# yewzijian/RegTR

Measured on NVIDIA H100. Metric: pairs/sec on 3DMatch-size clouds (~20k pts); pose err vs ref, higher is better.
Workload: dtype f32

## Files before the change

include/regtr_b200.h:

```cpp
#ifndef REGTR_B200_H_
#define REGTR_B200_H_

#include <stddef.h>
#include <stdint.h>

#ifdef __cplusplus
extern "C" {
#endif

#define REGTR_OK 0
#define REGTR_ERR_ARG (-1)
#define REGTR_ERR_WORKSPACE (-2)
#define REGTR_ERR_UNSUPPORTED (-3)

#define REGTR_STATUS_KEY_RANGE 1u
#define REGTR_STATUS_CAPACITY 2u
#define REGTR_STATUS_GRID 4u
#define REGTR_STATUS_RANGE 8u

int regtr_version(void);
const char* regtr_build_info(void);


size_t regtr_grid_subsample_ws_bytes(int n_cap, int n_clouds);
size_t regtr_grid_subsample_state_bytes(int n_cap);
int regtr_grid_subsample(const float* xyz, const int32_t* offs, int n_clouds, int n_cap, float dl,
                         float* out_xyz, int out_cap, int32_t* out_offs, uint32_t* status,
                         void* ws, size_t ws_bytes, void* state, size_t state_bytes, void* stream);
size_t regtr_grid_subsample_sorted_ws_bytes(int n_cap);
int regtr_grid_subsample_sorted(const float* xyz, const int32_t* offs, int n_clouds, int n_cap, float dl,
                                float* out_xyz, int out_cap, int32_t* out_offs, uint32_t* status,
                                void* ws, size_t ws_bytes, void* stream);

size_t regtr_cellgrid_bytes(int n_cap);
size_t regtr_cellgrid_ws_bytes(int n_cap);
size_t regtr_cellgrid_state_bytes(int n_cap);
int regtr_cellgrid_build(const float* xyz, const int32_t* offs, int n_clouds, int n_cap, float cell,
                         void* grid, int32_t* order, uint32_t* status,
                         void* ws, size_t ws_bytes, void* state, size_t state_bytes, void* stream);

int regtr_ball_query(const float* q, const int32_t* q_offs, const int32_t* q_order,
                     const float* s, const int32_t* s_offs, const void* s_grid,
                     int n_clouds, int nq_cap, int s_cap, int K, float radius,
                     int32_t* out_idx32, int64_t* out_idx64, void* stream);


size_t regtr_kpconv_ws_bytes(int Nq, int Ns, int Cin);
size_t regtr_kpconv_fwd_ws_bytes(int Nq, int Ns, int Cin, int Cout);
int regtr_kpconv_fwd(const float* q, const float* s, const int32_t* idx, const float* x,
                     const float* W, const float* kp, int Nq, int Ns, const int32_t* nq_dev,
                     const int32_t* ns_dev, int K, int Cin, int Cout,
                     float extent, float* out, void* ws, size_t ws_bytes, void* stream);

int regtr_kpconv_aggregate(const float* q, const float* s, const int32_t* idx, const float* x,
                           const float* kp, int Nq, int Ns, const int32_t* nq_dev, const int32_t* ns_dev,
                           int K, int Cin, float extent,
                           float* wf, uint8_t* rowflag_ws, int flags_ready, void* stream);

int regtr_max_pool(const float* x, const int32_t* idx, int Nq, int Ns, const int32_t* ns_dev, int K, int C,
                   float* out, void* stream);

size_t regtr_instnorm_ws_bytes(int n_cap, int n_clouds, int C);
size_t regtr_instnorm_counter_bytes(int n_clouds, int C);
int regtr_instnorm_act(const float* x, const int32_t* offs, int n_clouds, int n_cap, int C, float eps,
                       const float* res, float slope, float* out, uint8_t* rowflag_out,
                       void* ws, size_t ws_bytes, int32_t* counters, void* stream);

int regtr_instnorm_apply(const float* x, const int32_t* offs, int n_clouds, int n_cap, int C, const float* stats,
                         const float* res, float slope, float* out, uint8_t* rowflag_out, void* stream);


int regtr_split_tf32(const float* x, long long n, float* hi, float* lo, void* stream);

size_t regtr_gemm_ws_bytes(int M, int N, int K);
int regtr_gemm_tf32x3(const float* A, int lda, const float* B_hi, const float* B_lo, int ldb,
                      float* C, int ldc, const float* bias, const float* R, int ldr,
                      int M, int N, int K, const int32_t* m_dev, int relu,
                      void* ws, size_t ws_bytes, void* stream);

size_t regtr_instnorm_part_bytes(int M, int N);
int regtr_gemm_tf32x3_instats(const float* A, int lda, const float* B_hi, const float* B_lo, int ldb,
                              float* C, int ldc, int M, int N, int K, const int32_t* m_dev,
                              const int32_t* offs, int n_clouds, float eps, void* part, float* stats,
                              void* ws, size_t ws_bytes, void* stream);


int regtr_pos_embed_sine(const float* xyz, int n, const float* dim_t, int n_freq, int d_model,
                         float scale, float* out, void* stream);

int regtr_layernorm_pos(const float* x, const float* gamma, const float* beta, const float* pos,
                        int n, const int32_t* n_dev, int E, float eps, float* y, float* y_pos, void* stream);

int regtr_attention_plan(const int32_t* offs, int B, int32_t* plan, void* stream);

int regtr_mha_varlen_fwd(const float* Q, int ldq, const float* K, int ldk, const float* V, int ldv,
                         float* O, int ldo, const int32_t* q_start, const int32_t* q_len,
                         const int32_t* k_start, const int32_t* k_len, int n_problems,
                         int max_q_len, const int32_t* tile_base, int max_tiles,
                         int n_heads, int head_dim, float scale, void* stream);

int regtr_corr_decode_fwd(const float* Qp, const float* Kp, int ld, const float* xyz, float* out,
                          const int32_t* q_start, const int32_t* q_len, const int32_t* k_start,
                          const int32_t* k_len, int n_problems, int max_q_len, int n_layers, int n_rows,
                          int D, float scale, void* stream);

int regtr_gemm_tf32x3_qkv_bf16(const float* A, int lda, const float* B_hi, const float* B_lo, int ldb,
                               const float* bias, int M, int N, int K, int split, void* qk_out, int ld_qk,
                               void* vt_out, int ld_vt, const int32_t* m_dev, void* stream);
int regtr_mha_bf16_tc_fwd(const void* QK, int ld_qk, const void* Vt, int ld_vt, int n_tokens, float* O,
                          int ldo, const int32_t* q_start, const int32_t* q_len, const int32_t* k_start,
                          const int32_t* k_len, int n_problems, int max_q_len, int n_heads, int head_dim,
                          float scale, void* stream);

int regtr_gemm_tf32x3_qkv_split(const float* A, int lda, const float* B_hi, const float* B_lo, int ldb,
                                const float* bias, int M, int N, int K, int E, float qscale, float* qk4, int ld4,
                                float* vt2, int ld_vt, const int32_t* m_dev, void* stream);
int regtr_mha_tf32_tc_fwd(const float* qk4, int ld4, const float* vt2, int ld_vt, int n_tokens, float* O, int ldo,
                          const int32_t* q_start, const int32_t* q_len, const int32_t* k_start,
                          const int32_t* k_len, int n_problems, int max_q_len, const int32_t* tile_base,
                          int max_tiles, int n_heads, int head_dim, void* stream);

int regtr_mha_varlen_fwd_lse(const float* Q, int ldq, const float* K, int ldk, const float* V, int ldv,
// ... 175 lines not shown
```

regtr_b200/csrc/gemm_tc.cu:

```cuda
#include <cuda_bf16.h>


#include "common.cuh"
#include <stdlib.h>

#include "tc.cuh"

namespace {

struct QkvOut {
    __nv_bfloat16* qk;
    int ld_qk;
    __nv_bfloat16* vt;
    int ld_vt;
    int split;
    float* qk4;
    int ld4;
    float* vt2;
    int ld_vtf;
    int E;
    float qscale;
};
constexpr QkvOut NO_QKV = {nullptr, 0, nullptr, 0, 0, nullptr, 0, nullptr, 0, 0, 0.f};


template <int OFF>
__device__ __forceinline__ void transpose_sum_step(float (&v)[32], int lane) {
    const bool up = (lane & OFF) != 0;
#pragma unroll
    for (int i = 0; i < OFF; ++i) {
        const float mine = up ? v[i + OFF] : v[i];
        const float give = up ? v[i] : v[i + OFF];
        v[i] = mine + __shfl_xor_sync(0xffffffffu, give, OFF);
    }
    if constexpr (OFF > 1) transpose_sum_step<OFF / 2>(v, lane);
}
__device__ __forceinline__ float warp_transpose_sum(float (&v)[32], int lane) {
    transpose_sum_step<16>(v, lane);
    return v[0];
}

__global__ void __launch_bounds__(256)
k_in_finalize_part(const float2* __restrict__ part, const float* __restrict__ C, int ldc, const int32_t* __restrict__ offs,
                   int N, float eps, int direct_all, float2* __restrict__ stats) {
    __shared__ double red[8][32][2];
    const int c = blockIdx.x, col = blockIdx.y * 32 + threadIdx.x, w = threadIdx.y;
    const int a = offs[c], b = offs[c + 1];
    int g_lo = (a + 31) >> 5, g_hi = b >> 5;
    const bool full = !direct_all && g_lo < g_hi;
    const int head_end = full ? 32 * g_lo : b, tail_start = full ? 32 * g_hi : b;
    double s = 0.0, q = 0.0, k0 = 0.0;
    if (col < N && b > a) {
        k0 = (double)C[(size_t)a * ldc + col];
        if (full)
            for (int g = g_lo + w; g < g_hi; g += 8) {
                const float2 p = part[(size_t)g * N + col];
                const double d = (double)C[(size_t)g * 32 * ldc + col] - k0;
                s += (double)p.x + 32.0 * d;
                q += (double)p.y + d * (2.0 * (double)p.x + 32.0 * d);
            }
        for (int r = a + w; r < head_end; r += 8) { const double v = (double)C[(size_t)r * ldc + col] - k0; s += v; q += v * v; }
        for (int r = tail_start + w; r < b; r += 8) { const double v = (double)C[(size_t)r * ldc + col] - k0; s += v; q += v * v; }
    }
    red[w][threadIdx.x][0] = s; red[w][threadIdx.x][1] = q;
    __syncthreads();
    if (w == 0 && col < N) {
        for (int t = 1; t < 8; ++t) { s += red[t][threadIdx.x][0]; q += red[t][threadIdx.x][1]; }
        const int n = b - a;
        const double dn = n > 0 ? (double)n : 1.0;
        const double shift = s / dn;
        double var = q / dn - shift * shift;
        var = var > 0.0 ? var : 0.0;
        stats[(size_t)c * N + col] = make_float2((float)(k0 + shift), (float)(1.0 / sqrt(var + (double)eps)));
    }
}

constexpr int BM = 128;
constexpr int BK = 32;
constexpr uint32_t HI_MASK = 0xFFFFE000u;

__device__ __forceinline__ float tf32_hi(float x) { return regtr_tf32_rne(x); }

__global__ void k_split_tf32(const float* __restrict__ x, long long n, float* __restrict__ hi, float* __restrict__ lo) {
    const long long i = (long long)blockIdx.x * blockDim.x + threadIdx.x;
    if (i >= n) return;
    const float v = x[i], h = tf32_hi(v);
    hi[i] = h;
    lo[i] = tf32_hi(v - h);
}

constexpr int CONSUMER_THREADS = 256;
constexpr int GEMM_THREADS = CONSUMER_THREADS + 32;

template <int BN, int ST> struct CfgT {
    static constexpr int STAGES = ST;
    static constexpr int A_BYTES = BM * BK * 4;
    static constexpr int B_BYTES = BN * BK * 4;
    static constexpr int STAGE_BYTES = A_BYTES + 2 * B_BYTES;
    static constexpr int LDT = BN + 4;
    static constexpr int TILE_BYTES = BM * LDT * 4;
    static constexpr int SMEM = STAGES * STAGE_BYTES + TILE_BYTES + 1024  + 256 ;
    static constexpr int MIN_CTAS = SMEM <= 113 * 1024 ? 2 : 1;
};

__device__ __forceinline__ void consumer_sync() { asm volatile("bar.sync 1, %0;" ::"n"(CONSUMER_THREADS) : "memory"); }

template <int BN>
__device__ __forceinline__ void wgmma_tf32(float* d, const uint32_t* a, uint64_t bdesc, uint32_t accumulate) {
    if constexpr (BN == 128) tc::wgmma_tf32_n128(d, a, bdesc, accumulate);
    else if constexpr (BN == 64) tc::wgmma_tf32_n64(d, a, bdesc, accumulate);
    else tc::wgmma_tf32_n32(d, a, bdesc, accumulate);
}

template <int BN, int ST>
__global__ void __launch_bounds__(GEMM_THREADS, CfgT<BN, ST>::MIN_CTAS)
// ... 481 lines not shown
```

regtr_b200/csrc/norm.cu:

```cuda
#include "common.cuh"

namespace {

constexpr int IN_CH = 128;
constexpr int IN_TY = 8;
constexpr int IN_CT = 128;

__device__ __forceinline__ bool chunk_of(const int32_t* __restrict__ offs, int n_clouds, int chunk, int& cloud,
                                         int& r0, int& r1, int& first, int& count) {
    int acc = 0;
    for (int c = 0; c < n_clouds; ++c) {
        const int a = offs[c], b = offs[c + 1];
        const int nc = (b - a + IN_CH - 1) / IN_CH;
        if (chunk < acc + nc) {
            cloud = c;
            r0 = a + (chunk - acc) * IN_CH;
            r1 = min(r0 + IN_CH, b);
            first = acc;
            count = nc;
            return true;
        }
        acc += nc;
    }
    return false;
// ... 55 lines not shown
                fs[j] += p.x; fss[j] += p.y;
            }
    }
#pragma unroll
    for (int j = 0; j < 4; ++j) { red[threadIdx.y][threadIdx.x][j] = fs[j]; red[threadIdx.y][threadIdx.x][4 + j] = fss[j]; }
    __syncthreads();
    if (threadIdx.y == 0 && c < C) {
        for (int t = 1; t < IN_TY; ++t)
#pragma unroll
            for (int j = 0; j < 4; ++j) { fs[j] += red[t][threadIdx.x][j]; fss[j] += red[t][threadIdx.x][4 + j]; }
        const int n = offs[cloud + 1] - offs[cloud];
        const double dn = n > 0 ? (double)n : 1.0;
#pragma unroll
        for (int j = 0; j < 4; ++j) {
            const double mean = fs[j] / dn;
            double var = fss[j] / dn - mean * mean;
            var = var > 0.0 ? var : 0.0;
            stats[(size_t)cloud * C + c + j] = make_float2((float)mean, (float)(1.0 / sqrt(var + (double)eps)));
        }
    }
}

__global__ void __launch_bounds__(32 * IN_TY)
k_in_finalize(const int32_t* __restrict__ offs, int n_clouds, int C, float eps, const double2* __restrict__ partial,
              float2* __restrict__ stats) {
    __shared__ double2 red[IN_TY][32];
    const int cloud = blockIdx.x;
    const int c = blockIdx.y * 32 + threadIdx.x;
    int first = 0;
    for (int k = 0; k < cloud; ++k) first += (offs[k + 1] - offs[k] + IN_CH - 1) / IN_CH;
    const int n = offs[cloud + 1] - offs[cloud];
    const int nc = (n + IN_CH - 1) / IN_CH;
    double s = 0.0, ss = 0.0;
    if (c < C) {
        for (int t = threadIdx.y; t < nc; t += IN_TY) {
            const double2 p = partial[(size_t)(first + t) * C + c];
            s += p.x; ss += p.y;
        }
    }
    red[threadIdx.y][threadIdx.x] = make_double2(s, ss);
    __syncthreads();
    if (threadIdx.y == 0 && c < C) {
        for (int t = 1; t < IN_TY; ++t) { s += red[t][threadIdx.x].x; ss += red[t][threadIdx.x].y; }
        const double dn = n > 0 ? (double)n : 1.0;
        const double mean = s / dn;
        double var = ss / dn - mean * mean;
        var = var > 0.0 ? var : 0.0;
        stats[(size_t)cloud * C + c] = make_float2((float)mean, (float)(1.0 / sqrt(var + (double)eps)));
    }
}

template <bool FLAGS>
__global__ void k_in_apply(const float* x, const int32_t* __restrict__ offs, int n_clouds, int n_cap, int C,
                           const float2* __restrict__ stats, const float* res, float slope, float* out,
                           uint8_t* __restrict__ flags) {
    const int c4n = C >> 2;
    const int n_real = offs[n_clouds];
    const unsigned total = (unsigned)min(n_cap, (n_real + 127) & ~127) * (unsigned)c4n;
    const unsigned stride = gridDim.x * blockDim.x;
    for (unsigned t0 = blockIdx.x * blockDim.x; t0 < total; t0 += stride) {
        const unsigned t = t0 + threadIdx.x;
        const bool in_range = t < total;
        int r = 0, c = 0;
        if (in_range) { regtr_row_col(t, (unsigned)c4n, r, c); c *= 4; }
        const size_t o = (size_t)r * C + c;
        const bool live = in_range && r < n_real;
        float y[4] = {0.f, 0.f, 0.f, 0.f};
        if (live) {
            const float4 v = *reinterpret_cast<const float4*>(x + o);
            float4 rv = make_float4(0.f, 0.f, 0.f, 0.f);
            if (res) rv = *reinterpret_cast<const float4*>(res + o);
            const int cloud = regtr_cloud_of(offs, n_clouds, r);
            const float4 st01 = *reinterpret_cast<const float4*>(stats + (size_t)cloud * C + c);
            const float4 st23 = *reinterpret_cast<const float4*>(stats + (size_t)cloud * C + c + 2);
            y[0] = (v.x - st01.x) * st01.y + rv.x; y[1] = (v.y - st01.z) * st01.w + rv.y;
            y[2] = (v.z - st23.x) * st23.y + rv.z; y[3] = (v.w - st23.z) * st23.w + rv.w;
            if (slope >= 0.f) {
#pragma unroll
                for (int j = 0; j < 4; ++j) y[j] = y[j] > 0.f ? y[j] : y[j] * slope;
            }
        }
        if (in_range) *reinterpret_cast<float4*>(out + o) = make_float4(y[0], y[1], y[2], y[3]);
        if (FLAGS) {
            double acc = ((double)y[0] + (double)y[1]) + ((double)y[2] + (double)y[3]);
            for (int d = 1; d < c4n; d <<= 1) acc += __shfl_xor_sync(0xffffffffu, acc, d);
            if (in_range && (threadIdx.x & (c4n - 1)) == 0) flags[r] = live && acc > 0.0;
        }
    }
}

template <int PER>
__global__ void k_layernorm_pos(const float* __restrict__ x, const float* __restrict__ gamma,
                                const float* __restrict__ beta, const float* __restrict__ pos, int n,
                                const int32_t* __restrict__ n_dev, int E, float eps, float* __restrict__ y,
                                float* __restrict__ y_pos) {
    const int row = (blockIdx.x * blockDim.x + threadIdx.x) >> 5, lane = threadIdx.x & 31;
    if (n_dev) n = min(n, *n_dev);
    if (row >= n) return;
    const float* xr = x + (size_t)row * E;
    const int per = E / 32;
    float v[PER], gm[PER], bt[PER], ps[PER];
#pragma unroll
    for (int j = 0; j < PER; ++j)
        if (j < per) {
            const int c = j * 32 + lane;
            v[j] = xr[c]; gm[j] = __ldg(gamma + c); bt[j] = __ldg(beta + c);
            ps[j] = (y_pos && pos) ? pos[(size_t)row * E + c] : 0.f;
        }
    float s = 0.f;
#pragma unroll
    for (int j = 0; j < PER; ++j) if (j < per) s += v[j];
    const float mean = warp_sum(s) / (float)E;
    float ss = 0.f;
#pragma unroll
    for (int j = 0; j < PER; ++j) if (j < per) { const float d = v[j] - mean; ss += d * d; }
    const float rstd = 1.f / sqrtf(warp_sum(ss) / (float)E + eps);
#pragma unroll
    for (int j = 0; j < PER; ++j) {
        if (j >= per) break;
        const int c = j * 32 + lane;
        const float o = (v[j] - mean) * rstd * gm[j] + bt[j];
        if (y) y[(size_t)row * E + c] = o;
        if (y_pos) y_pos[(size_t)row * E + c] = o + ps[j];
    }
}
// ... 6 lines not shown
    regtr_row_col((unsigned)t, (unsigned)d_model, i, c);
    float o = 0.f;
    if (c < 3 * n_freq) {
        const int a = c / n_freq, f = c % n_freq;
        const float v = __fdiv_rn(__fmul_rn(xyz[3 * i + a], scale), dim_t[f]);
        o = (f & 1) ? cosf(v) : sinf(v);
    }
    out[t] = o;
}

static inline int in_apply_grid(long long items) {
    const long long b = (items + 255) / 256;
    return (int)(b < 8 * REGTR_NUM_SMS ? (b > 0 ? b : 1) : 8 * REGTR_NUM_SMS);
}

}

extern "C" {

static inline int in_chunks(int n_cap, int n_clouds) { return regtr_cdiv(n_cap > 0 ? n_cap : 1, IN_CH) + n_clouds; }

size_t regtr_instnorm_ws_bytes(int n_cap, int n_clouds, int C) {
    const size_t c = (size_t)(C > 0 ? C : 1), nc = (size_t)(n_clouds > 0 ? n_clouds : 1);
    return regtr_align((size_t)in_chunks(n_cap, (int)nc) * c * sizeof(double2)) + regtr_align(nc * c * sizeof(float2));
}

size_t regtr_instnorm_counter_bytes(int n_clouds, int C) {
    return sizeof(int32_t) * (size_t)(n_clouds > 0 ? n_clouds : 1) * (size_t)regtr_cdiv(C > 0 ? C : 1, IN_CT);
}

int regtr_instnorm_act(const float* x, const int32_t* offs, int n_clouds, int n_cap, int C, float eps,
                       const float* res, float slope, float* out, uint8_t* rowflag_out, void* ws, size_t ws_bytes,
                       int32_t* counters, void* stream_) {
    cudaStream_t st = (cudaStream_t)stream_;
    if (!offs || n_clouds <= 0 || n_cap < 0 || C <= 0) return REGTR_ERR_ARG;
    if (C % 4 != 0 || (long long)n_cap * (C / 4) >= (1ll << 31)) return REGTR_ERR_UNSUPPORTED;
    if (n_cap == 0) return REGTR_OK;
    if (!x || !out || !ws) return REGTR_ERR_ARG;
    if (ws_bytes < regtr_instnorm_ws_bytes(n_cap, n_clouds, C)) return REGTR_ERR_WORKSPACE;
    const int chunks = in_chunks(n_cap, n_clouds);
    double2* partial = (double2*)ws;
    float2* stats = (float2*)((char*)ws + regtr_align((size_t)chunks * C * sizeof(double2)));
    dim3 block(32, IN_TY);
    k_in_stats<<<dim3(chunks, regtr_cdiv(C, IN_CT)), block, 0, st>>>(x, offs, n_clouds, C, partial, counters, eps, stats);
    REGTR_CHECK_LAUNCH();
    if (!counters) {
        k_in_finalize<<<dim3(n_clouds, regtr_cdiv(C, 32)), block, 0, st>>>(offs, n_clouds, C, eps, partial, stats);
        REGTR_CHECK_LAUNCH();
    }
    if (rowflag_out) {
        const int c4n = C / 4;
        if (c4n > 32 || (c4n & (c4n - 1))) return REGTR_ERR_UNSUPPORTED;
        k_in_apply<true><<<in_apply_grid((long long)n_cap * c4n), 256, 0, st>>>(x, offs, n_clouds, n_cap, C, stats,
                                                                                  res, slope, out, rowflag_out);
    } else {
        k_in_apply<false><<<in_apply_grid((long long)n_cap * (C / 4)), 256, 0, st>>>(x, offs, n_clouds, n_cap, C,
                                                                                      stats, res, slope, out, nullptr);
    }
    REGTR_CHECK_LAUNCH();
    return REGTR_OK;
}

int regtr_instnorm_apply(const float* x, const int32_t* offs, int n_clouds, int n_cap, int C, const float* stats,
                         const float* res, float slope, float* out, uint8_t* rowflag_out, void* stream_) {
    cudaStream_t st = (cudaStream_t)stream_;
    if (!offs || n_clouds <= 0 || n_cap < 0 || C <= 0) return REGTR_ERR_ARG;
    if (C % 4 != 0 || (long long)n_cap * (C / 4) >= (1ll << 31)) return REGTR_ERR_UNSUPPORTED;
    if (n_cap == 0) return REGTR_OK;
    if (!x || !out || !stats) return REGTR_ERR_ARG;
    const float2* stp = reinterpret_cast<const float2*>(stats);
    if (rowflag_out) {
        const int c4n = C / 4;
        if (c4n > 32 || (c4n & (c4n - 1))) return REGTR_ERR_UNSUPPORTED;
        k_in_apply<true><<<in_apply_grid((long long)n_cap * c4n), 256, 0, st>>>(x, offs, n_clouds, n_cap, C, stp, res, slope,
                                                                                  out, rowflag_out);
    } else {
        k_in_apply<false><<<in_apply_grid((long long)n_cap * (C / 4)), 256, 0, st>>>(x, offs, n_clouds, n_cap, C, stp, res,
                                                                                      slope, out, nullptr);
    }
    REGTR_CHECK_LAUNCH();
    return REGTR_OK;
}

int regtr_layernorm_pos(const float* x, const float* gamma, const float* beta, const float* pos, int n,
                        const int32_t* n_dev, int E, float eps, float* y, float* y_pos, void* stream_) {
    cudaStream_t st = (cudaStream_t)stream_;
    if (n < 0 || E <= 0 || E % 32 != 0 || E > 1024) return REGTR_ERR_ARG;
    if (n == 0) return REGTR_OK;
    if (!x || !gamma || !beta || (!y && !y_pos)) return REGTR_ERR_ARG;
    if (E <= 256)
        k_layernorm_pos<8><<<regtr_cdiv((long long)n * 32, 256), 256, 0, st>>>(x, gamma, beta, pos, n, n_dev, E, eps, y, y_pos);
    else
        k_layernorm_pos<32><<<regtr_cdiv((long long)n * 32, 256), 256, 0, st>>>(x, gamma, beta, pos, n, n_dev, E, eps, y, y_pos);
    REGTR_CHECK_LAUNCH();
    return REGTR_OK;
}

int regtr_pos_embed_sine(const float* xyz, int n, const float* dim_t, int n_freq, int d_model, float scale,
                         float* out, void* stream_) {
    cudaStream_t st = (cudaStream_t)stream_;
    if (n < 0 || n_freq <= 0 || d_model < 3 * n_freq) return REGTR_ERR_ARG;
    if ((long long)n * d_model >= (1ll << 31)) return REGTR_ERR_UNSUPPORTED;
    if (n == 0) return REGTR_OK;
    if (!xyz || !dim_t || !out) return REGTR_ERR_ARG;
    k_pos_embed_sine<<<regtr_cdiv((long long)n * d_model, 256), 256, 0, st>>>(xyz, n, dim_t, n_freq, d_model, scale, out);
    REGTR_CHECK_LAUNCH();
    return REGTR_OK;
}

}
```

regtr_b200/kpconv.py:

```python
from __future__ import annotations

import logging
from typing import List

import torch
import torch.nn as nn
import torch.nn.functional as F

from . import ops
from .config import pyramid_plan
from .lazy import LazyDict
from .weights import kernel_disposition

_CELL_SLACK = 1.0001



def level_capacities(cfg, cap0: int, ratio: float = 0.40, quantum: int = 256):
    levels, _, _ = pyramid_plan(cfg)
    caps = [int(cap0)]
    for _ in levels[1:]:
        c = int(caps[-1] * ratio) + 1
        caps.append(min(caps[-1], (c + quantum - 1) // quantum * quantum))
    return caps
# ... 167 lines not shown
    return ops.max_pool(x.contiguous(), inds if inds.dtype == torch.int32 else inds.to(torch.int32))


class KPConv(nn.Module):

    def __init__(self, kernel_size, p_dim, in_channels, out_channels, KP_extent, radius,
                 fixed_kernel_points='center', KP_influence='linear', aggregation_mode='sum',
                 deformable=False, modulated=False):
        super().__init__()
        if deformable or modulated:
            raise NotImplementedError('deformable / modulated KPConv is outside the hot path')
        if KP_influence != 'linear' or aggregation_mode != 'sum':
            raise NotImplementedError("only KP_influence='linear', aggregation_mode='sum' are on the hot path")
        if kernel_size != 15 or p_dim != 3:
            raise NotImplementedError('the fused kernel is specialised for 15 kernel points in 3-D')
        self.K, self.p_dim = kernel_size, p_dim
        self.in_channels, self.out_channels = in_channels, out_channels
        self.radius, self.KP_extent = radius, KP_extent
        self.weights = nn.Parameter(torch.empty((kernel_size, in_channels, out_channels), dtype=torch.float32))
        bound = 1.0 / (in_channels * out_channels) ** 0.5
        nn.init.uniform_(self.weights, -bound, bound)
        self.kernel_points = nn.Parameter(torch.from_numpy(kernel_disposition(radius, kernel_size)),
                                          requires_grad=False)

    def forward(self, q_pts, s_pts, neighb_inds, x, nq_dev=None, ns_dev=None, row_flags=None, instats=None):
        idx = neighb_inds if neighb_inds.dtype == torch.int32 else neighb_inds.to(torch.int32)
        return ops.kpconv(q_pts.contiguous(), s_pts.contiguous(), idx.contiguous(), x.contiguous(),
                          self.weights, self.kernel_points, self.KP_extent, nq_dev=nq_dev, ns_dev=ns_dev,
                          row_flags=row_flags, instats=instats)

    def __repr__(self):
        return 'KPConv(radius: {:.2f}, extent: {:.2f}, in_feat: {:d}, out_feat: {:d})'.format(
            self.radius, self.KP_extent, self.in_channels, self.out_channels)


class BatchNormBlock(nn.Module):

    def __init__(self, in_dim, use_bn, bn_momentum):
        super().__init__()
        self.in_dim, self.use_bn, self.bn_momentum = in_dim, use_bn, bn_momentum
        if not use_bn:
            self.bias = nn.Parameter(torch.zeros(in_dim, dtype=torch.float32))

    def fuse(self, x, offs, n_clouds, res=None, slope=-1.0, want_flags=False):
        if self.use_bn:
            return ops.instnorm_act(x, offs, n_clouds, res=res, slope=slope, want_flags=want_flags)
        if want_flags:
            raise NotImplementedError('row flags are only fused into the InstanceNorm pass')
        y = x + self.bias
        if res is not None:
            y = y + res
        return F.leaky_relu(y, slope) if slope >= 0 else y

    def apply(self, x, stats, offs, n_clouds, res=None, slope=-1.0, want_flags=False):
        return ops.instnorm_apply(x, offs, n_clouds, stats, res=res, slope=slope, want_flags=want_flags)

    def forward(self, x, stack_lengths):
        offs = ops.make_offsets(stack_lengths, x.device)
        return self.fuse(x.contiguous(), offs, offs.numel() - 1)


class UnaryBlock(nn.Module):

    def __init__(self, in_dim, out_dim, use_bn, bn_momentum, no_relu=False):
        super().__init__()
        self.in_dim, self.out_dim, self.use_bn, self.no_relu = in_dim, out_dim, use_bn, no_relu
        self.mlp = nn.Linear(in_dim, out_dim, bias=False)
        self.batch_norm = BatchNormBlock(out_dim, use_bn, bn_momentum)

    def fuse(self, x, offs, n_clouds, res=None, final_slope=None, m_dev=None, want_flags=False, skip=False):
        slope = final_slope if final_slope is not None else (-1.0 if self.no_relu else 0.1)
        if self.use_bn and self.out_dim % 32 == 0 and EPILOGUE_STATS:
            y, stats, *xs = ops.linear_instats(x, self.mlp.weight, offs, n_clouds, m_dev=m_dev, skip=skip)
            out = self.batch_norm.apply(y, stats, offs, n_clouds, res=res, slope=slope, want_flags=want_flags)
        else:
            xs = [x]
            out = self.batch_norm.fuse(ops.linear(x, self.mlp.weight, m_dev=m_dev), offs, n_clouds, res=res,
                                       slope=slope, want_flags=want_flags)
        if not skip:
            return out
        return (*out, xs[0]) if want_flags else (out, xs[0])

    def forward(self, x, stack_lengths=None):
        offs = ops.make_offsets(stack_lengths, x.device)
        return self.fuse(x, offs, offs.numel() - 1)


def _block_io(block, batch):
    m = _meta_private(batch, batch['points'][0].device if 'points' in batch else batch['_points'][0].device)
    li = block.layer_ind
    pts, offs, nd = m['_points'], m['_offs'], m['_ndev']
    if 'strided' in block.block_name:
        return (pts[li + 1], pts[li], m['_pools32'][li], offs[li], offs[li + 1],
                nd[li + 1] if nd else None, nd[li] if nd else None, m['_n_clouds'])
    return (pts[li], pts[li], m['_neighbors32'][li], offs[li], offs[li],
            nd[li] if nd else None, nd[li] if nd else None, m['_n_clouds'])


class SimpleBlock(nn.Module):

    def __init__(self, block_name, in_dim, out_dim, radius, layer_ind, config):
        super().__init__()
        self.block_name, self.layer_ind = block_name, layer_ind
        self.in_dim, self.out_dim = in_dim, out_dim
        extent = radius * config.KP_extent / config.conv_radius
        self.KPConv = KPConv(config.num_kernel_points, config.in_points_dim, in_dim, out_dim // 2, extent, radius,
                             fixed_kernel_points=config.fixed_kernel_points, KP_influence=config.KP_influence,
                             aggregation_mode=config.aggregation_mode, deformable='deform' in block_name,
                             modulated=config.modulated)
        self.batch_norm = BatchNormBlock(out_dim // 2, config.use_batch_norm, config.batch_norm_momentum)

    def forward(self, x, batch):
        q, s, idx, _, offs_post, nq_dev, ns_dev, nc = _block_io(self, batch)
        y = self.KPConv(q, s, idx, x, nq_dev, ns_dev)
        return self.batch_norm.fuse(y, offs_post, nc, slope=0.1)


class ResnetBottleneckBlock(nn.Module):

    def __init__(self, block_name, in_dim, out_dim, radius, layer_ind, config):
        super().__init__()
        self.block_name, self.layer_ind = block_name, layer_ind
        self.in_dim, self.out_dim = in_dim, out_dim
        bn, mom = config.use_batch_norm, config.batch_norm_momentum
        self.use_bn = bn
        extent = radius * config.KP_extent / config.conv_radius
        mid = out_dim // 4
        self.unary1 = UnaryBlock(in_dim, mid, bn, mom) if in_dim != mid else nn.Identity()
        self.KPConv = KPConv(config.num_kernel_points, config.in_points_dim, mid, mid, extent, radius,
                             fixed_kernel_points=config.fixed_kernel_points, KP_influence=config.KP_influence,
                             aggregation_mode=config.aggregation_mode, deformable='deform' in block_name,
                             modulated=config.modulated)
        self.batch_norm_conv = BatchNormBlock(mid, bn, mom)
        self.unary2 = UnaryBlock(mid, out_dim, bn, mom, no_relu=True)
        self.unary_shortcut = UnaryBlock(in_dim, out_dim, bn, mom, no_relu=True) if in_dim != out_dim \
            else nn.Identity()

    def forward(self, features, batch):
        q, s, idx, offs_pre, offs_post, nq_dev, ns_dev, nc = _block_io(self, batch)
        flags = None
        if isinstance(self.unary1, UnaryBlock) and self.use_bn:
            x, flags, features = self.unary1.fuse(features, offs_pre, nc, m_dev=ns_dev, want_flags=True, skip=True)
        else:
            x = self.unary1.fuse(features, offs_pre, nc, m_dev=ns_dev) if isinstance(self.unary1, UnaryBlock) \
                else features
        if self.use_bn and self.KPConv.out_channels % 32 == 0 and EPILOGUE_STATS:
            x, stats = self.KPConv(q, s, idx, x, nq_dev, ns_dev, row_flags=flags, instats=(offs_post, nc))
            x = self.batch_norm_conv.apply(x, stats, offs_post, nc, slope=0.1)
        else:
            x = self.KPConv(q, s, idx, x, nq_dev, ns_dev, row_flags=flags)
            x = self.batch_norm_conv.fuse(x, offs_post, nc, slope=0.1)
        shortcut = ops.max_pool(features, idx, ns_dev) if 'strided' in self.block_name else features
        if isinstance(self.unary_shortcut, UnaryBlock):
            shortcut = self.unary_shortcut.fuse(shortcut, offs_post, nc, m_dev=nq_dev)
        return self.unary2.fuse(x, offs_post, nc, res=shortcut, final_slope=0.1, m_dev=nq_dev)


def block_decider(block_name, radius, in_dim, out_dim, layer_ind, config):
    if block_name in ('simple', 'simple_strided'):
        return SimpleBlock(block_name, in_dim, out_dim, radius, layer_ind, config)
    if block_name in ('resnetb', 'resnetb_strided'):
        return ResnetBottleneckBlock(block_name, in_dim, out_dim, radius, layer_ind, config)
    raise NotImplementedError(f'block {block_name!r} is outside the RegTR hot path (SURVEY.md 2 row 3)')


class KPFEncoder(nn.Module):

    def __init__(self, config, d_bottle, increase_channel_when_downsample=True):
        super().__init__()
        self.logger = logging.getLogger(__name__)
        octave = 0
        r = config.first_subsampling_dl * config.conv_radius
        in_dim, out_dim = config.in_feats_dim, config.first_feats_dim
        self.encoder_blocks = nn.ModuleList()
        self.encoder_skip_dims, self.encoder_skips = [], []
        block = None
        for block_i, block in enumerate(config.architecture):
            if any(t in block for t in ('pool', 'strided', 'upsample', 'global')):
                self.encoder_skips.append(block_i)
                self.encoder_skip_dims.append(in_dim)
            if 'upsample' in block:
                break
            self.encoder_blocks.append(block_decider(block, r, in_dim, out_dim, octave, config))
            in_dim = out_dim // 2 if 'simple' in block else out_dim
            if 'pool' in block or 'strided' in block:
                octave += 1
                r *= 2
                if increase_channel_when_downsample:
                    out_dim *= 2
        if 'upsample' not in block:
            self.encoder_skips.append(block_i)
            self.encoder_skip_dims.append(in_dim)

    def forward(self, x, batch):
        skip_x = []
        for block_i, block_op in enumerate(self.encoder_blocks):
            if block_i in self.encoder_skips:
                skip_x.append(x)
            x = block_op(x, batch)
        return x, skip_x
```

regtr_b200/lib.py:

```python
from __future__ import annotations

import ctypes
import os
import re

import torch

HERE = os.path.dirname(os.path.abspath(__file__))
LIB_PATH = os.path.join(HERE, 'libregtr_b200.so')
HEADER = os.path.join(os.path.dirname(HERE), 'include', 'regtr_b200.h')


class RegtrLibError(RuntimeError):
    pass


_c = ctypes
_P = _c.c_void_p
_I = _c.c_int
_F = _c.c_float
_Z = _c.c_size_t

SIGNATURES = {
    'regtr_version': (_I, []),
    'regtr_build_info': (_c.c_char_p, []),
    'regtr_grid_subsample_ws_bytes': (_Z, [_I, _I]),
    'regtr_grid_subsample_state_bytes': (_Z, [_I]),
    'regtr_grid_subsample': (_I, [_P, _P, _I, _I, _F, _P, _I, _P, _P, _P, _Z, _P, _Z, _P]),
    'regtr_grid_subsample_sorted_ws_bytes': (_Z, [_I]),
    'regtr_grid_subsample_sorted': (_I, [_P, _P, _I, _I, _F, _P, _I, _P, _P, _P, _Z, _P]),
    'regtr_cellgrid_bytes': (_Z, [_I]),
    'regtr_cellgrid_ws_bytes': (_Z, [_I]),
    'regtr_cellgrid_state_bytes': (_Z, [_I]),
    'regtr_cellgrid_build': (_I, [_P, _P, _I, _I, _F, _P, _P, _P, _P, _Z, _P, _Z, _P]),
    'regtr_ball_query': (_I, [_P, _P, _P, _P, _P, _P, _I, _I, _I, _I, _F, _P, _P, _P]),
    'regtr_kpconv_ws_bytes': (_Z, [_I, _I, _I]),
    'regtr_kpconv_fwd_ws_bytes': (_Z, [_I, _I, _I, _I]),
    'regtr_kpconv_fwd': (_I, [_P, _P, _P, _P, _P, _P, _I, _I, _P, _P, _I, _I, _I, _F, _P, _P, _Z, _P]),
    'regtr_kpconv_aggregate': (_I, [_P, _P, _P, _P, _P, _I, _I, _P, _P, _I, _I, _F, _P, _P, _I, _P]),
    'regtr_max_pool': (_I, [_P, _P, _I, _I, _P, _I, _I, _P, _P]),
    'regtr_instnorm_ws_bytes': (_Z, [_I, _I, _I]),
    'regtr_instnorm_counter_bytes': (_Z, [_I, _I]),
    'regtr_instnorm_act': (_I, [_P, _P, _I, _I, _I, _F, _P, _F, _P, _P, _P, _Z, _P, _P]),
    'regtr_instnorm_apply': (_I, [_P, _P, _I, _I, _I, _P, _P, _F, _P, _P, _P]),
    'regtr_instnorm_part_bytes': (_Z, [_I, _I]),
    'regtr_gemm_tf32x3_instats': (_I, [_P, _I, _P, _P, _I, _P, _I, _I, _I, _I, _P, _P, _I, _F, _P, _P, _P, _Z, _P]),
    'regtr_split_tf32': (_I, [_P, _c.c_longlong, _P, _P, _P]),
    'regtr_gemm_ws_bytes': (_Z, [_I, _I, _I]),
    'regtr_gemm_tf32x3': (_I, [_P, _I, _P, _P, _I, _P, _I, _P, _P, _I, _I, _I, _I, _P, _I, _P, _Z, _P]),
    'regtr_pos_embed_sine': (_I, [_P, _I, _P, _I, _I, _F, _P, _P]),
    'regtr_layernorm_pos': (_I, [_P, _P, _P, _P, _I, _P, _I, _F, _P, _P, _P]),
    'regtr_attention_plan': (_I, [_P, _I, _P, _P]),
    'regtr_corr_decode_fwd': (_I, [_P, _P, _I, _P, _P, _P, _P, _P, _P, _I, _I, _I, _I, _I, _F, _P]),
    'regtr_mha_varlen_fwd': (_I, [_P, _I, _P, _I, _P, _I, _P, _I, _P, _P, _P, _P, _I, _I, _P, _I, _I, _I, _F, _P]),
    'regtr_gemm_tf32x3_qkv_bf16': (_I, [_P, _I, _P, _P, _I, _P, _I, _I, _I, _I, _P, _I, _P, _I, _P, _P]),
    'regtr_mha_bf16_tc_fwd': (_I, [_P, _I, _P, _I, _I, _P, _I, _P, _P, _P, _P, _I, _I, _I, _I, _F, _P]),
    'regtr_gemm_tf32x3_qkv_split': (_I, [_P, _I, _P, _P, _I, _P, _I, _I, _I, _I, _F, _P, _I, _P, _I, _P, _P]),
    'regtr_mha_tf32_tc_fwd': (_I, [_P, _I, _P, _I, _I, _P, _I, _P, _P, _P, _P, _I, _I, _P, _I, _I, _I, _P]),
    'regtr_mha_varlen_fwd_lse': (_I, [_P, _I, _P, _I, _P, _I, _P, _I, _P, _P, _P, _P, _P, _I, _I, _I, _I, _F, _P]),
    'regtr_mha_varlen_bwd_ws_bytes': (_Z, [_I, _I]),
    'regtr_mha_varlen_bwd': (_I, [_P, _I, _P, _I, _P, _I, _P, _I, _P, _I, _P, _P, _I, _P, _I, _P, _I,
                                  _P, _P, _P, _P, _I, _I, _I, _I, _I, _I, _F, _P, _Z, _P]),
    'regtr_layernorm_bwd_ws_bytes': (_Z, [_I, _I]),
    'regtr_layernorm_bwd': (_I, [_P, _P, _P, _P, _P, _I, _I, _F, _P, _P, _P, _P, _Z, _P]),
    'regtr_relu_bwd': (_I, [_P, _P, _c.c_longlong, _P, _P]),
    'regtr_linear_wgrad_ws_bytes': (_Z, [_I, _I, _I]),
    'regtr_linear_wgrad': (_I, [_P, _I, _P, _I, _I, _I, _I, _P, _P, _P, _Z, _P]),
    'regtr_neighbor_csr_ws_bytes': (_Z, [_I]),
    'regtr_neighbor_csr': (_I, [_P, _I, _I, _I, _P, _P, _P, _Z, _P]),
    'regtr_kpconv_bwd_input_ws_bytes': (_Z, [_I, _I, _I]),
    'regtr_kpconv_bwd_input': (_I, [_P, _P, _P, _P, _P, _P, _I, _I, _I, _I, _F, _P, _P, _P, _P, _P, _Z, _P]),
    'regtr_max_pool_bwd_ws_bytes': (_Z, [_I, _I]),
    'regtr_max_pool_bwd': (_I, [_P, _P, _I, _I, _I, _I, _P, _P, _P, _P, _P, _Z, _P]),
    'regtr_instnorm_bwd_ws_bytes': (_Z, [_I, _I, _I]),
    'regtr_instnorm_bwd': (_I, [_P, _P, _P, _P, _I, _I, _I, _F, _F, _P, _P, _P, _Z, _P]),
    'regtr_grad_norm_ws_bytes': (_Z, [_I]),
    'regtr_grad_norm': (_I, [_P, _I, _I, _F, _P, _P, _Z, _P]),
    'regtr_grad_scale': (_I, [_P, _I, _I, _P, _P]),
    'regtr_adam_step': (_I, [_P, _I, _I, _P]),
    'regtr_split_refresh': (_I, [_P, _I, _I, _P]),
    'regtr_kabsch_fwd': (_I, [_P, _P, _P, _P, _I, _P, _P]),
    'regtr_pose_from_corr': (_I, [_P, _P, _P, _P, _I, _I, _I, _P, _P]),
    'regtr_overlap_coord_bound': (_c.c_double, [_c.c_double, _F]),
    'regtr_overlap_ws_bytes': (_Z, [_I]),
    'regtr_overlap_state_bytes': (_Z, [_I]),
    'regtr_overlap_nn': (_I, [_P, _P, _I, _I, _P, _c.c_double, _F, _P, _P, _P, _Z, _P, _Z, _P]),
    'regtr_registration_fit': (_I, [_P, _P, _I, _I, _P, _c.c_double, _P, _P, _P, _P]),
    'regtr_train_augment_ws_bytes': (_Z, [_I, _I]),
    'regtr_train_augment_state_bytes': (_Z, [_I]),
    'regtr_train_augment': (_I, [_P, _P, _I, _I, _P, _P, _P, _P, _c.c_ulonglong, _c.c_ulonglong, _c.c_double, _I,
                                 _P, _I, _P, _P, _P, _P, _I, _P, _P, _Z, _P, _Z, _P]),
    'regtr_meter_update': (_I, [_P, _P]),
    'regtr_pose_errors': (_I, [_P, _P]),
    'regtr_modelnet_augment': (_I, [_P, _P]),
    'regtr_status_clear': (_I, [_P, _P]),
}

# ... 46 lines not shown
```

regtr_b200/ops.py:

```python
from __future__ import annotations

import contextlib
import itertools
import math

import numpy as np
import torch

from . import lib as _lib

_ws_cache = {}

LAUNCHES = 0
KPCONV_TRACE = None
TRACE = None


def _count(n):
    global LAUNCHES
    LAUNCHES += n


def _stream():
    return torch.cuda.current_stream().cuda_stream
# ... 208 lines not shown
    return wf


def max_pool(x, idx32, ns_dev=None):
    if _wants_grad(x):
        if ns_dev is not None:
            raise ValueError('max_pool: the backward needs exact shapes (no ns_dev)')
        return _MaxPoolFn.apply(x, idx32)
    return _max_pool_fwd(x, idx32, ns_dev)


def _max_pool_fwd(x, idx32, ns_dev=None):
    L = _lib.load()
    _chk(x, torch.float32, 'x', 2); _chk(idx32, torch.int32, 'inds', 2)
    Nq, K = idx32.shape
    out = torch.empty((Nq, x.shape[1]), dtype=torch.float32, device=x.device)
    _lib.check(L.regtr_max_pool(_p(x), _p(idx32), Nq, x.shape[0], _p(ns_dev), K, x.shape[1], _p(out), _stream()),
               'regtr_max_pool')
    _count(1)
    return out


def instnorm_act(x, offs, n_clouds: int, res=None, slope: float = -1.0, eps: float = 1e-5, out=None,
                 want_flags: bool = False):
    if _wants_grad(x, res):
        if out is not None:
            raise ValueError('instnorm_act: no out= on the differentiable path')
        y, flags = _InstNormFn.apply(x, res, None, offs, n_clouds, float(slope), float(eps), bool(want_flags))
        return (y, flags) if want_flags else y
    return _instnorm_act_fwd(x, offs, n_clouds, res, slope, eps, out, want_flags)


def _instnorm_act_fwd(x, offs, n_clouds: int, res=None, slope: float = -1.0, eps: float = 1e-5, out=None,
                      want_flags: bool = False):
    L = _lib.load()
    _chk(x, torch.float32, 'x', 2); _chk(offs, torch.int32, 'offs', 1)
    n, C = x.shape
    if res is not None:
        _chk(res, torch.float32, 'res', 2)
    out = torch.empty_like(x) if out is None else out
    nb = L.regtr_instnorm_ws_bytes(n, n_clouds, C)
    ws = workspace(nb, x.device, 'instnorm')
    flags = None
    if want_flags and C // 4 <= 32 and (C // 4) & (C // 4 - 1) == 0:
        flags = torch.empty(max(n, 1), dtype=torch.uint8, device=x.device)
    cnt = workspace(L.regtr_instnorm_counter_bytes(n_clouds, C), x.device, 'instnorm_cnt', zero=True)
    _lib.check(L.regtr_instnorm_act(_p(x), _p(offs), n_clouds, n, C, float(eps), _p(res), float(slope), _p(out),
                                    _p(flags), _p(ws), ws.numel(), _p(cnt), _stream()), 'regtr_instnorm_act')
    _count(2)
    return (out, flags) if want_flags else out


def instnorm_apply(x, offs, n_clouds: int, stats, res=None, slope: float = -1.0, out=None, want_flags: bool = False,
                   eps: float = 1e-5):
    if _wants_grad(x, res):
        if out is not None:
            raise ValueError('instnorm_apply: no out= on the differentiable path')
        y, flags = _InstNormFn.apply(x, res, stats, offs, n_clouds, float(slope), float(eps), bool(want_flags))
        return (y, flags) if want_flags else y
    return _instnorm_apply_fwd(x, offs, n_clouds, stats, res, slope, out, want_flags)


def _instnorm_apply_fwd(x, offs, n_clouds: int, stats, res=None, slope: float = -1.0, out=None,
                        want_flags: bool = False):
    L = _lib.load()
    _chk(x, torch.float32, 'x', 2); _chk(offs, torch.int32, 'offs', 1); _chk(stats, torch.float32, 'stats', 3)
    n, C = x.shape
    out = torch.empty_like(x) if out is None else out
    flags = None
    if want_flags and C // 4 <= 32 and (C // 4) & (C // 4 - 1) == 0:
        flags = torch.empty(max(n, 1), dtype=torch.uint8, device=x.device)
    _lib.check(L.regtr_instnorm_apply(_p(x), _p(offs), n_clouds, n, C, _p(stats), _p(res), float(slope), _p(out),
                                      _p(flags), _stream()), 'regtr_instnorm_apply')
    _count(1)
    return (out, flags) if want_flags else out



def split_weight(w: torch.Tensor, transpose: bool = False):
    L = _lib.load()
    owner = w._base if w._base is not None else w
    cache = owner.__dict__.setdefault('_regtr_split', {})
    key = (w.storage_offset(), tuple(w.shape), tuple(w.stride()), transpose, owner._version)
    hit = cache.get(key)
    if hit is not None:
        return hit
    src = (w.detach().t() if transpose else w.detach()).contiguous().to(torch.float32)
    hi, lo = torch.empty_like(src), torch.empty_like(src)
    _lib.check(L.regtr_split_tf32(_p(src), src.numel(), _p(hi), _p(lo), _stream()), 'regtr_split_tf32')
    _count(1)
    for k in [k for k in cache if k[-1] != owner._version]:
        del cache[k]
    cache[key] = (hi, lo)
    return hi, lo


def gemm(a, b_hi, b_lo, bias=None, residual=None, relu=False, m_dev=None, out=None):
    L = _lib.load()
    if not a.is_cuda or a.dtype != torch.float32 or a.dim() != 2 or a.stride(1) != 1:
        raise ValueError('gemm: A must be a CUDA fp32 matrix with unit column stride')
    M, K = a.shape
    N = b_hi.shape[0]
    out = torch.empty((M, N), dtype=torch.float32, device=a.device) if out is None else out
    nb = L.regtr_gemm_ws_bytes(M, N, K)
    ws = workspace(nb, a.device, 'gemm')
    if TRACE is not None:
        TRACE.append(('gemm', dict(M=M, N=N, K=K, split_k=nb > 256),
                      lambda: gemm(a, b_hi, b_lo, bias=bias, residual=residual, relu=relu, m_dev=m_dev, out=out)))
    _lib.check(L.regtr_gemm_tf32x3(_p(a), a.stride(0), _p(b_hi), _p(b_lo), b_hi.stride(0), _p(out), out.stride(0),
                                   _p(bias), _p(residual), residual.stride(0) if residual is not None else 0,
                                   M, N, K, _p(m_dev), 1 if relu else 0, _p(ws), ws.numel(), _stream()),
               'regtr_gemm_tf32x3')
    _count(2 if nb > 256 else 1)
    return out


def gemm_instats(a, b_hi, b_lo, offs, n_clouds: int, eps: float = 1e-5, m_dev=None, out=None):
    L = _lib.load()
    if not a.is_cuda or a.dtype != torch.float32 or a.dim() != 2 or a.stride(1) != 1:
        raise ValueError('gemm: A must be a CUDA fp32 matrix with unit column stride')
    M, K = a.shape
    N = b_hi.shape[0]
    out = torch.empty((M, N), dtype=torch.float32, device=a.device) if out is None else out
    stats = torch.empty((n_clouds, N, 2), dtype=torch.float32, device=a.device)
    nb = L.regtr_gemm_ws_bytes(M, N, K)
    ws = workspace(nb, a.device, 'gemm')
# ... 726 lines not shown
```

Baseline: 862.0.

## Fuse shortcut instance-norm into residual apply and unroll finalize loads

The unary shortcut branch no longer runs its own instance-norm apply kernel. Its GEMM now produces only the statistics, and the residual is normalized on the fly inside the final apply kernel by passing res_stats. This removes one elementwise kernel launch and a full read/write pass over the shortcut tensor for each residual block. Separately, the stats finalize kernel unrolls its row loads eight-wide so more loads are in flight. The cost is extra stat loads in the apply kernel and more API surface to keep consistent.

After: 880.7, median of 6. No clear change (+2.2%).

```diff
diff --git a/include/regtr_b200.h b/include/regtr_b200.h
--- a/include/regtr_b200.h
+++ b/include/regtr_b200.h
@@ -67,7 +67,8 @@
                        void* ws, size_t ws_bytes, int32_t* counters, void* stream);
 
 int regtr_instnorm_apply(const float* x, const int32_t* offs, int n_clouds, int n_cap, int C, const float* stats,
-                         const float* res, float slope, float* out, uint8_t* rowflag_out, void* stream);
+                         const float* res, const float* res_stats, float slope, float* out, uint8_t* rowflag_out,
+                         void* stream);
 
 
 int regtr_split_tf32(const float* x, long long n, float* hi, float* lo, void* stream);
diff --git a/regtr_b200/csrc/gemm_tc.cu b/regtr_b200/csrc/gemm_tc.cu
--- a/regtr_b200/csrc/gemm_tc.cu
+++ b/regtr_b200/csrc/gemm_tc.cu
@@ -40,6 +40,8 @@
     return v[0];
 }
 
+constexpr int FIN_U = 8;
+
 __global__ void __launch_bounds__(256)
 k_in_finalize_part(const float2* __restrict__ part, const float* __restrict__ C, int ldc, const int32_t* __restrict__ offs,
                    int N, float eps, int direct_all, float2* __restrict__ stats) {
@@ -50,17 +52,39 @@
     const bool full = !direct_all && g_lo < g_hi;
     const int head_end = full ? 32 * g_lo : b, tail_start = full ? 32 * g_hi : b;
     double s = 0.0, q = 0.0, k0 = 0.0;
+    auto add_rows = [&](int r0, int r1) {
+        for (int r = r0 + w; r < r1; r += 8 * FIN_U) {
+            float v[FIN_U];
+#pragma unroll
+            for (int u = 0; u < FIN_U; ++u)
+                if (r + 8 * u < r1) v[u] = C[(size_t)(r + 8 * u) * ldc + col];
+#pragma unroll
+            for (int u = 0; u < FIN_U; ++u)
+                if (r + 8 * u < r1) { const double d = (double)v[u] - k0; s += d; q += d * d; }
+        }
+    };
     if (col < N && b > a) {
         k0 = (double)C[(size_t)a * ldc + col];
         if (full)
-            for (int g = g_lo + w; g < g_hi; g += 8) {
-                const float2 p = part[(size_t)g * N + col];
-                const double d = (double)C[(size_t)g * 32 * ldc + col] - k0;
-                s += (double)p.x + 32.0 * d;
-                q += (double)p.y + d * (2.0 * (double)p.x + 32.0 * d);
-            }
-        for (int r = a + w; r < head_end; r += 8) { const double v = (double)C[(size_t)r * ldc + col] - k0; s += v; q += v * v; }
-        for (int r = tail_start + w; r < b; r += 8) { const double v = (double)C[(size_t)r * ldc + col] - k0; s += v; q += v * v; }
+            for (int g = g_lo + w; g < g_hi; g += 8 * FIN_U) {
+                float2 p[FIN_U];
+                float v[FIN_U];
+#pragma unroll
+                for (int u = 0; u < FIN_U; ++u)
+                    if (g + 8 * u < g_hi) {
+                        p[u] = part[(size_t)(g + 8 * u) * N + col];
+                        v[u] = C[(size_t)(g + 8 * u) * 32 * ldc + col];
+                    }
+#pragma unroll
+                for (int u = 0; u < FIN_U; ++u)
+                    if (g + 8 * u < g_hi) {
+                        const double d = (double)v[u] - k0;
+                        s += (double)p[u].x + 32.0 * d;
+                        q += (double)p[u].y + d * (2.0 * (double)p[u].x + 32.0 * d);
+                    }
+            }
+        add_rows(a, head_end);
+        add_rows(tail_start, b);
     }
     red[w][threadIdx.x][0] = s; red[w][threadIdx.x][1] = q;
     __syncthreads();
diff --git a/regtr_b200/csrc/norm.cu b/regtr_b200/csrc/norm.cu
--- a/regtr_b200/csrc/norm.cu
+++ b/regtr_b200/csrc/norm.cu
@@ -131,8 +131,8 @@
 
 template <bool FLAGS>
 __global__ void k_in_apply(const float* x, const int32_t* __restrict__ offs, int n_clouds, int n_cap, int C,
-                           const float2* __restrict__ stats, const float* res, float slope, float* out,
-                           uint8_t* __restrict__ flags) {
+                           const float2* __restrict__ stats, const float* res, const float2* __restrict__ res_stats,
+                           float slope, float* out, uint8_t* __restrict__ flags) {
     const int c4n = C >> 2;
     const int n_real = offs[n_clouds];
     const unsigned total = (unsigned)min(n_cap, (n_real + 127) & ~127) * (unsigned)c4n;
@@ -150,6 +150,14 @@
             float4 rv = make_float4(0.f, 0.f, 0.f, 0.f);
             if (res) rv = *reinterpret_cast<const float4*>(res + o);
             const int cloud = regtr_cloud_of(offs, n_clouds, r);
+            if (res_stats) {
+                const float4 rs01 = *reinterpret_cast<const float4*>(res_stats + (size_t)cloud * C + c);
+                const float4 rs23 = *reinterpret_cast<const float4*>(res_stats + (size_t)cloud * C + c + 2);
+                rv.x = __fadd_rn(__fmul_rn(__fsub_rn(rv.x, rs01.x), rs01.y), 0.f);
+                rv.y = __fadd_rn(__fmul_rn(__fsub_rn(rv.y, rs01.z), rs01.w), 0.f);
+                rv.z = __fadd_rn(__fmul_rn(__fsub_rn(rv.z, rs23.x), rs23.y), 0.f);
+                rv.w = __fadd_rn(__fmul_rn(__fsub_rn(rv.w, rs23.z), rs23.w), 0.f);
+            }
             const float4 st01 = *reinterpret_cast<const float4*>(stats + (size_t)cloud * C + c);
             const float4 st23 = *reinterpret_cast<const float4*>(stats + (size_t)cloud * C + c + 2);
             y[0] = (v.x - st01.x) * st01.y + rv.x; y[1] = (v.y - st01.z) * st01.w + rv.y;
@@ -262,31 +270,33 @@
         const int c4n = C / 4;
         if (c4n > 32 || (c4n & (c4n - 1))) return REGTR_ERR_UNSUPPORTED;
         k_in_apply<true><<<in_apply_grid((long long)n_cap * c4n), 256, 0, st>>>(x, offs, n_clouds, n_cap, C, stats,
-                                                                                  res, slope, out, rowflag_out);
+                                                                                  res, nullptr, slope, out, rowflag_out);
     } else {
         k_in_apply<false><<<in_apply_grid((long long)n_cap * (C / 4)), 256, 0, st>>>(x, offs, n_clouds, n_cap, C,
-                                                                                      stats, res, slope, out, nullptr);
+                                                                                      stats, res, nullptr, slope, out, nullptr);
     }
     REGTR_CHECK_LAUNCH();
     return REGTR_OK;
 }
 
 int regtr_instnorm_apply(const float* x, const int32_t* offs, int n_clouds, int n_cap, int C, const float* stats,
-                         const float* res, float slope, float* out, uint8_t* rowflag_out, void* stream_) {
+                         const float* res, const float* res_stats, float slope, float* out, uint8_t* rowflag_out,
+                         void* stream_) {
     cudaStream_t st = (cudaStream_t)stream_;
     if (!offs || n_clouds <= 0 || n_cap < 0 || C <= 0) return REGTR_ERR_ARG;
     if (C % 4 != 0 || (long long)n_cap * (C / 4) >= (1ll << 31)) return REGTR_ERR_UNSUPPORTED;
     if (n_cap == 0) return REGTR_OK;
-    if (!x || !out || !stats) return REGTR_ERR_ARG;
+    if (!x || !out || !stats || (res_stats && !res)) return REGTR_ERR_ARG;
     const float2* stp = reinterpret_cast<const float2*>(stats);
+    const float2* rsp = reinterpret_cast<const float2*>(res_stats);
     if (rowflag_out) {
         const int c4n = C / 4;
         if (c4n > 32 || (c4n & (c4n - 1))) return REGTR_ERR_UNSUPPORTED;
-        k_in_apply<true><<<in_apply_grid((long long)n_cap * c4n), 256, 0, st>>>(x, offs, n_clouds, n_cap, C, stp, res, slope,
-                                                                                  out, rowflag_out);
+        k_in_apply<true><<<in_apply_grid((long long)n_cap * c4n), 256, 0, st>>>(x, offs, n_clouds, n_cap, C, stp, res, rsp,
+                                                                                  slope, out, rowflag_out);
     } else {
         k_in_apply<false><<<in_apply_grid((long long)n_cap * (C / 4)), 256, 0, st>>>(x, offs, n_clouds, n_cap, C, stp, res,
-                                                                                      slope, out, nullptr);
+                                                                                      rsp, slope, out, nullptr);
     }
     REGTR_CHECK_LAUNCH();
     return REGTR_OK;
diff --git a/regtr_b200/kpconv.py b/regtr_b200/kpconv.py
--- a/regtr_b200/kpconv.py
+++ b/regtr_b200/kpconv.py
@@ -243,8 +243,9 @@
             y = y + res
         return F.leaky_relu(y, slope) if slope >= 0 else y
 
-    def apply(self, x, stats, offs, n_clouds, res=None, slope=-1.0, want_flags=False):
-        return ops.instnorm_apply(x, offs, n_clouds, stats, res=res, slope=slope, want_flags=want_flags)
+    def apply(self, x, stats, offs, n_clouds, res=None, res_stats=None, slope=-1.0, want_flags=False):
+        return ops.instnorm_apply(x, offs, n_clouds, stats, res=res, res_stats=res_stats, slope=slope,
+                                  want_flags=want_flags)
 
     def forward(self, x, stack_lengths):
         offs = ops.make_offsets(stack_lengths, x.device)
@@ -259,12 +260,19 @@
         self.mlp = nn.Linear(in_dim, out_dim, bias=False)
         self.batch_norm = BatchNormBlock(out_dim, use_bn, bn_momentum)
 
-    def fuse(self, x, offs, n_clouds, res=None, final_slope=None, m_dev=None, want_flags=False, skip=False):
+    @property
+    def epilogue_stats(self):
+        return self.use_bn and self.out_dim % 32 == 0 and EPILOGUE_STATS
+
+    def fuse(self, x, offs, n_clouds, res=None, res_stats=None, final_slope=None, m_dev=None, want_flags=False,
+             skip=False):
         slope = final_slope if final_slope is not None else (-1.0 if self.no_relu else 0.1)
-        if self.use_bn and self.out_dim % 32 == 0 and EPILOGUE_STATS:
+        if self.epilogue_stats:
             y, stats, *xs = ops.linear_instats(x, self.mlp.weight, offs, n_clouds, m_dev=m_dev, skip=skip)
-            out = self.batch_norm.apply(y, stats, offs, n_clouds, res=res, slope=slope, want_flags=want_flags)
+            out = self.batch_norm.apply(y, stats, offs, n_clouds, res=res, res_stats=res_stats, slope=slope,
+                                        want_flags=want_flags)
         else:
+            assert res_stats is None
             xs = [x]
             out = self.batch_norm.fuse(ops.linear(x, self.mlp.weight, m_dev=m_dev), offs, n_clouds, res=res,
                                        slope=slope, want_flags=want_flags)
@@ -342,9 +350,14 @@
             x = self.KPConv(q, s, idx, x, nq_dev, ns_dev, row_flags=flags)
             x = self.batch_norm_conv.fuse(x, offs_post, nc, slope=0.1)
         shortcut = ops.max_pool(features, idx, ns_dev) if 'strided' in self.block_name else features
+        res_stats = None
         if isinstance(self.unary_shortcut, UnaryBlock):
-            shortcut = self.unary_shortcut.fuse(shortcut, offs_post, nc, m_dev=nq_dev)
-        return self.unary2.fuse(x, offs_post, nc, res=shortcut, final_slope=0.1, m_dev=nq_dev)
+            if self.unary_shortcut.epilogue_stats:
+                shortcut, res_stats = ops.linear_instats(shortcut, self.unary_shortcut.mlp.weight, offs_post, nc,
+                                                         m_dev=nq_dev)
+            else:
+                shortcut = self.unary_shortcut.fuse(shortcut, offs_post, nc, m_dev=nq_dev)
+        return self.unary2.fuse(x, offs_post, nc, res=shortcut, res_stats=res_stats, final_slope=0.1, m_dev=nq_dev)
 
 
 def block_decider(block_name, radius, in_dim, out_dim, layer_ind, config):
diff --git a/regtr_b200/lib.py b/regtr_b200/lib.py
--- a/regtr_b200/lib.py
+++ b/regtr_b200/lib.py
@@ -42,7 +42,7 @@
     'regtr_instnorm_ws_bytes': (_Z, [_I, _I, _I]),
     'regtr_instnorm_counter_bytes': (_Z, [_I, _I]),
     'regtr_instnorm_act': (_I, [_P, _P, _I, _I, _I, _F, _P, _F, _P, _P, _P, _Z, _P, _P]),
-    'regtr_instnorm_apply': (_I, [_P, _P, _I, _I, _I, _P, _P, _F, _P, _P, _P]),
+    'regtr_instnorm_apply': (_I, [_P, _P, _I, _I, _I, _P, _P, _P, _F, _P, _P, _P]),
     'regtr_instnorm_part_bytes': (_Z, [_I, _I]),
     'regtr_gemm_tf32x3_instats': (_I, [_P, _I, _P, _P, _I, _P, _I, _I, _I, _I, _P, _P, _I, _F, _P, _P, _P, _Z, _P]),
     'regtr_split_tf32': (_I, [_P, _c.c_longlong, _P, _P, _P]),
diff --git a/regtr_b200/ops.py b/regtr_b200/ops.py
--- a/regtr_b200/ops.py
+++ b/regtr_b200/ops.py
@@ -284,26 +284,32 @@
 
 
 def instnorm_apply(x, offs, n_clouds: int, stats, res=None, slope: float = -1.0, out=None, want_flags: bool = False,
-                   eps: float = 1e-5):
+                   eps: float = 1e-5, res_stats=None):
     if _wants_grad(x, res):
         if out is not None:
             raise ValueError('instnorm_apply: no out= on the differentiable path')
+        if res_stats is not None:
+            res = instnorm_apply(res, offs, n_clouds, res_stats, eps=eps)
         y, flags = _InstNormFn.apply(x, res, stats, offs, n_clouds, float(slope), float(eps), bool(want_flags))
         return (y, flags) if want_flags else y
-    return _instnorm_apply_fwd(x, offs, n_clouds, stats, res, slope, out, want_flags)
+    return _instnorm_apply_fwd(x, offs, n_clouds, stats, res, slope, out, want_flags, res_stats)
 
 
 def _instnorm_apply_fwd(x, offs, n_clouds: int, stats, res=None, slope: float = -1.0, out=None,
-                        want_flags: bool = False):
+                        want_flags: bool = False, res_stats=None):
     L = _lib.load()
     _chk(x, torch.float32, 'x', 2); _chk(offs, torch.int32, 'offs', 1); _chk(stats, torch.float32, 'stats', 3)
     n, C = x.shape
+    if res is not None and (_chk(res, torch.float32, 'res', 2).shape != x.shape):
+        raise ValueError('instnorm_apply: res must have the shape of x')
+    if res_stats is not None and (res is None or _chk(res_stats, torch.float32, 'res_stats', 3).shape != stats.shape):
+        raise ValueError('instnorm_apply: res_stats needs res and the shape of stats')
     out = torch.empty_like(x) if out is None else out
     flags = None
     if want_flags and C // 4 <= 32 and (C // 4) & (C // 4 - 1) == 0:
         flags = torch.empty(max(n, 1), dtype=torch.uint8, device=x.device)
-    _lib.check(L.regtr_instnorm_apply(_p(x), _p(offs), n_clouds, n, C, _p(stats), _p(res), float(slope), _p(out),
-                                      _p(flags), _stream()), 'regtr_instnorm_apply')
+    _lib.check(L.regtr_instnorm_apply(_p(x), _p(offs), n_clouds, n, C, _p(stats), _p(res), _p(res_stats), float(slope),
+                                      _p(out), _p(flags), _stream()), 'regtr_instnorm_apply')
     _count(1)
     return (out, flags) if want_flags else out
 
```
